# kjyv/FloBaRoID

Hardware: AMD Instinct MI355X
Metric: regressor samples/s (fused regressor->Gram pass) + TSQR TFLOP/s, WALK-MAN 31-DOF float-base (higher is better)
Workload: dtype f64

## Files before the change

flobaroid_amd/csrc/fbr_gram64.h:

```cpp
#pragma once
#define FBR_G64_SWZ(c) (2 * ((c) & 15))
#include <algorithm>
#include <type_traits>
#include <utility>

#include "fbr_kinid.h"

struct FbrGram64Tile {
    int col[FBR_TILE];
    std::vector<int> path;
    int friction = 0;
    int lo = 0, hi = 0;
};

struct FbrGram64 {
    int NT = 0;
    int NF = 0;
    int nlev = 0, fb = 0, flev = 0, ntr = 0, maxact = 0, npw = 0, wpb = 8;
    long blk_doubles = 0;
    std::vector<int> trow;
    std::vector<int> slab;
    int nstage = 0, base_stages = 0;
    std::vector<int> stage_lev;
    std::vector<int> lev_begin;
// ... 444 lines not shown
        for (int pq = 0; pq < pr.nparts; pq++)
            if (own[pq][l]) {
                pr.rel[((size_t)pq * hm.L + l) * FBR_G64_WORDS + 14 + p] = word(tr0, sl);
                pr.lcol[(size_t)pr.nparts * 10 * hm.L + ((size_t)pq * hm.L + l) * FBR_G64_FRIC + p] = c;
            }
    }
    pr.steps.clear();
    pr.nslots = 1;
    for (int pq = 0; pq < pr.nparts; pq++) {
        pr.step0[pq] = (int)(pr.steps.size() / FBR_KINID_STEP);
        pr.nsteps[pq] = progs[pq].nsteps;
        pr.nslots = std::max(pr.nslots, progs[pq].nslots);
        pr.steps.insert(pr.steps.end(), progs[pq].steps.begin(), progs[pq].steps.begin() + (size_t)progs[pq].nsteps * FBR_KINID_STEP);
    }
    return true;
}

static inline bool fbr_gram64_build_producer(const FbrHostModel &hm, const FbrGramProgram &, const FbrGram64 &g, FbrGram64Producer &pr)
{
    return fbr_gram64_build_producer(hm, g, pr);
}

#define FBR_G64_MAXK 2
FBR_HD int fbr_gram64_mom_count(int cols, int k) { return k * cols + k * (k + 1) / 2; }
FBR_HD void fbr_gram64_mom_target(int cols, int k, int idx, int *row, int *col)
{
    if (idx < k * cols) {
        *row = idx % cols;
        *col = cols + idx / cols;
        return;
    }
    int e = idx - k * cols, i = 0;
    while (e >= k - i) e -= k - i, i++;
    *row = cols + i;
    *col = cols + i + e;
}

#if defined(__HIPCC__) && defined(FBR_KERNELS_GRAM)
struct DevGram64 {
    int NT, nlev, maxact, npieces, nstage;
    long blk_doubles;
    const int *slab, *lev_begin, *pieces, *wmeta, *stage_lev;
    const int *runs;
};

template <int MAXD, bool HASW, int KR = 1>
__global__ __launch_bounds__(64 * FBR_KINWRITE_PARTS, MAXD <= 10 ? 2 : 1) void fbr_kinimg_kernel(DevModel m, DevKinId p, DevKinWrite wr, long S, long blk_doubles,
                                                                              const double *__restrict__ q, const double *__restrict__ dq,
                                                                              const double *__restrict__ ddq, const double *__restrict__ bv,
                                                                              const double *__restrict__ ba, const double *__restrict__ rpy,
                                                                              const double *__restrict__ rhs, const double *__restrict__ wts,
                                                                              double *__restrict__ scratch, double *__restrict__ mom,
                                                                              const double *__restrict__ sign)
{
    extern __shared__ __attribute__((aligned(16))) double smem[];
    const int lane = threadIdx.x & 63, part = __builtin_amdgcn_readfirstlane(threadIdx.x >> 6), nth = blockDim.x, tid = threadIdx.x;
    const int n = m.n, ldn = p.ldn, ldw = m.rows | 1, rows = m.rows;
    double *sq = smem, *sdq = sq + 64 * ldn, *sddq = sdq + 64 * ldn, *sw = sddq + 64 * ldn;
    double *st = sw + (HASW ? 64 * ldw : 0);
    double *scr = scratch + ((long)blockIdx.x * wr.nparts + part) * p.nslots * FBR_LINK_REC * 64 + lane;
    double *mo = mom ? mom + (long)blockIdx.x * (KR * wr.cols + KR * (KR + 1) / 2) * 64 : nullptr;
    const long Sg = wr.group_samples > 0 ? wr.group_samples : S, bpg = (Sg + 63) >> 6;
    const long nblk = (S / Sg) * bpg;
    const fbr_clong_ptr cdst = (fbr_clong_ptr)(unsigned long)wr.dst;
    const fbr_cint_ptr ccol = (fbr_cint_ptr)(unsigned long)(wr.lcol10 + (long)part * 10 * m.L);
    for (long blk = blockIdx.x; blk < nblk; blk += gridDim.x) {
        const long grp = blk / bpg, lb = blk - grp * bpg;
        const long base = grp * Sg + (lb << 6);
        const int valid = (int)min(64L, Sg - (lb << 6));
        __syncthreads();
        {
            const long off = base * n;
            const int cnt = valid * n;
            int sr = tid / n, dc = tid - sr * n;
            const int ds = nth / n, dd = nth - ds * n;
            for (int i = tid; i < cnt; i += nth) {
                const double a = q[off + i], b = dq[off + i], c = ddq[off + i];
                sq[sr * ldn + dc] = a;
                sdq[sr * ldn + dc] = b;
                sddq[sr * ldn + dc] = c;
                sr += ds;
                dc += dd;
                if (dc >= n) {
                    dc -= n;
                    sr++;
                }
            }
            if (HASW || wr.k) {
// ... 32 lines not shown
        };
        auto basest = [&](double *v6, double *a6, double *e3) {
            for (int i = 0; i < 6; i++) {
                v6[i] = bv[s * 6 + i];
                a6[i] = ba[s * 6 + i];
            }
            for (int i = 0; i < 3; i++) e3[i] = rpy[s * 3 + i];
        };
        auto save = [&](int b, int i, double v) { scr[(b * FBR_LINK_REC + i) * 64] = v; };
        auto load = [&](int b, int i) { return scr[(b * FBR_LINK_REC + i) * 64]; };
        auto consts = [&](int l, double *rR, double *rp, double *ax) {
            const fbr_cdouble_ptr cR = (fbr_cdouble_ptr)(unsigned long)m.restR, cp = (fbr_cdouble_ptr)(unsigned long)m.restp,
                                  ca = (fbr_cdouble_ptr)(unsigned long)m.axis;
            for (int i = 0; i < 9; i++) rR[i] = cR[9 * l + i];
            for (int i = 0; i < 3; i++) {
                rp[i] = cp[3 * l + i];
                ax[i] = ca[3 * l + i];
            }
        };
        const unsigned vlane = (unsigned)(((unsigned long)slot_off + (unsigned long)s31) << 3);
        auto link = [&](int l, int depth, const double *rec, const double (*Sst)[6], const int *lvd, double *F) {
            (void)F;
            if (wr.base_only) depth = 0;
            __builtin_amdgcn_s_waitcnt(0x0F70);
            long d10[10], dF[4];
#pragma unroll
            for (int pp = 0; pp < 10; pp++) d10[pp] = cdst[((long)part * m.L + l) * FBR_G64_WORDS + pp];
#pragma unroll
            for (int pp = 0; pp < 4; pp++) dF[pp] = cdst[((long)part * m.L + l) * FBR_G64_WORDS + 10 + pp];
            auto ft_of = [&](int ro, double *F) {
#pragma unroll
                for (int i = 0; i < 6; i++)
                    if (i < m.fb) F[i] = myt[ro + i];
#pragma unroll
                for (int j = 0; j < MAXD; j++)
                    if (j < depth) {
                        const double tj = myt[ro + m.fb + lvd[j]];
#pragma unroll
                        for (int i = 0; i < 6; i++) F[i] += Sst[j][i] * tj;
                    }
            };
            double Ft[6] = {0.0, 0.0, 0.0, 0.0, 0.0, 0.0};
            if constexpr (KR == 1) {
                if (wr.k) {
#pragma unroll
                    for (int i = 0; i < 6; i++)
                        if (i < m.fb) Ft[i] = myt[i];
#pragma unroll
                    for (int j = 0; j < MAXD; j++)
                        if (j < depth) {
                            const double tj = myt[m.fb + lvd[j]];
#pragma unroll
                            for (int i = 0; i < 6; i++) Ft[i] += Sst[j][i] * tj;
                        }
                }
            }
            auto ft_group = [&](int r, double *F) {
                int ro = r * 64 * ldw;
                asm volatile("" : "+v"(ro));
#pragma unroll
                for (int i = 0; i < 6; i++) F[i] = 0.0;
                ft_of(ro, F);
            };
            auto store = [&](long d0, int lv, double v) {
                if (d0 == 0) return;
                const unsigned vo = vlane ^ ((unsigned)(d0 & 0xff) << 3);
                __builtin_nontemporal_store(v, (fbr_gdouble_ptr)((fbr_gchar_ptr)(d0 & ~0xffL) + (long)lv * 8192 + vo));
            };
            auto full_group = [&](auto q0c, auto nqc) {
                constexpr int Q0 = decltype(q0c)::value, NQ = decltype(nqc)::value;
                double wA[NQ][6];
#pragma unroll
                for (int qq = 0; qq < NQ; qq++) fbr_unit_wrench(rec, Q0 + qq, wA[qq]);
#pragma unroll
                for (int i = 0; i < 6; i++)
                    if (i < m.fb) {
#pragma unroll
                        for (int qq = 0; qq < NQ; qq++) store(i < wr.flev ? dF[Q0 + qq] : d10[Q0 + qq], i, HASW ? wA[qq][i] * myw[i] : wA[qq][i]);
                    }
#pragma unroll
                for (int j = 0; j < MAXD; j++)
                    if (j < depth) {
                        double v[NQ];
#pragma unroll
                        for (int qq = 0; qq < NQ; qq++) v[qq] = fbr_dot6(Sst[j], wA[qq]);
                        const double wj = HASW ? myw[m.fb + lvd[j]] : 1.0;
#pragma unroll
                        for (int qq = 0; qq < NQ; qq++) store(d10[Q0 + qq], m.fb + j, HASW ? v[qq] * wj : v[qq]);
                    }
                if constexpr (KR == 1) {
                    if (wr.k) {
#pragma unroll
                        for (int qq = 0; qq < NQ; qq++)
                            if (d10[Q0 + qq]) unsafeAtomicAdd(mo + (long)ccol[10 * l + Q0 + qq] * 64 + lane, fbr_dot6(Ft, wA[qq]));
                    }
                } else {
#pragma unroll
                    for (int r = 0; r < KR; r++) {
                        double F[6];
                        ft_group(r, F);
#pragma unroll
                        for (int qq = 0; qq < NQ; qq++)
                            if (d10[Q0 + qq]) unsafeAtomicAdd(mo + ((long)r * wr.cols + ccol[10 * l + Q0 + qq]) * 64 + lane, fbr_dot6(F, wA[qq]));
                    }
                }
            };
            auto moment_group = [&](auto q0c, auto nqc) {
                constexpr int Q0 = decltype(q0c)::value, NQ = decltype(nqc)::value;
                double nB[NQ][3];
#pragma unroll
                for (int qq = 0; qq < NQ; qq++) fbr_unit_moment3(rec, 4 + Q0 + qq, nB[qq]);
#pragma unroll
                for (int i = 3; i < 6; i++)
                    if (i < m.fb) {
#pragma unroll
                        for (int qq = 0; qq < NQ; qq++) store(d10[4 + Q0 + qq], i, HASW ? nB[qq][i - 3] * myw[i] : nB[qq][i - 3]);
                    }
#pragma unroll
                for (int j = 0; j < MAXD; j++)
                    if (j < depth) {
                        double v[NQ];
#pragma unroll
                        for (int qq = 0; qq < NQ; qq++) v[qq] = Sst[j][3] * nB[qq][0] + Sst[j][4] * nB[qq][1] + Sst[j][5] * nB[qq][2];
                        const double wj = HASW ? myw[m.fb + lvd[j]] : 1.0;
#pragma unroll
                        for (int qq = 0; qq < NQ; qq++) store(d10[4 + Q0 + qq], m.fb + j, HASW ? v[qq] * wj : v[qq]);
                    }
                if constexpr (KR == 1) {
                    if (wr.k) {
#pragma unroll
                        for (int qq = 0; qq < NQ; qq++)
                            if (d10[4 + Q0 + qq])
                                unsafeAtomicAdd(mo + (long)ccol[10 * l + 4 + Q0 + qq] * 64 + lane, Ft[3] * nB[qq][0] + Ft[4] * nB[qq][1] + Ft[5] * nB[qq][2]);
                    }
                } else {
#pragma unroll
                    for (int r = 0; r < KR; r++) {
                        double F[6];
                        ft_group(r, F);
#pragma unroll
                        for (int qq = 0; qq < NQ; qq++)
                            if (d10[4 + Q0 + qq])
                                unsafeAtomicAdd(mo + ((long)r * wr.cols + ccol[10 * l + 4 + Q0 + qq]) * 64 + lane,
                                                F[3] * nB[qq][0] + F[4] * nB[qq][1] + F[5] * nB[qq][2]);
                    }
                }
            };
            using std::integral_constant;
            if constexpr (MAXD > 8 && MAXD <= 10) {
                full_group(integral_constant<int, 0>{}, integral_constant<int, 2>{});
                full_group(integral_constant<int, 2>{}, integral_constant<int, 2>{});
                moment_group(integral_constant<int, 0>{}, integral_constant<int, 3>{});
                moment_group(integral_constant<int, 3>{}, integral_constant<int, 3>{});
            } else {
                full_group(integral_constant<int, 0>{}, integral_constant<int, 4>{});
                moment_group(integral_constant<int, 0>{}, integral_constant<int, 6>{});
            }
            const int nfr = wr.cols > wr.ninert ? (wr.cols - wr.ninert) / n : 0;
            const int dj = nfr ? m.dof[l] : -1;
            if (dj >= 0 && depth > 0) {
                const fbr_cint_ptr cfr = (fbr_cint_ptr)(unsigned long)(wr.lcol10 + (long)wr.nparts * 10 * m.L + ((long)part * m.L + l) * FBR_G64_FRIC);
#pragma unroll
                for (int pf = 0; pf < FBR_G64_FRIC; pf++)
                    if (pf < nfr) {
                        const long dfw = cdst[((long)part * m.L + l) * FBR_G64_WORDS + 14 + pf];
                        if (dfw == 0) continue;
                        const int c = cfr[pf];
                        const double fv = fbr_friction_value(m.coldesc[c].z, mysdq[dj], sign ? sign[s * n + dj] : 0.0, m.stribeck);
                        store(dfw, m.fb + depth - 1, HASW ? fv * myw[m.fb + dj] : fv);
                        if constexpr (KR == 1) {
                            if (wr.k) unsafeAtomicAdd(mo + (long)c * 64 + lane, fv * myt[m.fb + dj]);
                        } else {
#pragma unroll
                            for (int r = 0; r < KR; r++) unsafeAtomicAdd(mo + ((long)r * wr.cols + c) * 64 + lane, fv * myt[r * 64 * ldw + m.fb + dj]);
                        }
                    }
            }
        };
        auto emit = [&](int, double) {};
        if (live) {
            fbr_kinid_lane<MAXD, false>(wr.part_nsteps[part], p.maxlvl, p.steps + wr.part_step0[part] * FBR_KINID_STEP, p.endflush, m.floating, m.g, m.fb,
                                        state, basest, save, load, link, emit, consts);
            if constexpr (KR == 1) {
                if (wr.k && part == wr.nparts - 1) {
                    double tt = 0.0;
                    for (int r = 0; r < rows; r++) {
                        const double wv = HASW ? myw[r] : 1.0, tv = rhs[s * rows + r] * wv;
                        tt += tv * tv;
                    }
                    unsafeAtomicAdd(mo + (long)wr.cols * 64 + lane, tt);
                }
            } else if (part == wr.nparts - 1) {
                double tt[KR * (KR + 1) / 2];
#pragma unroll
                for (int e = 0; e < KR * (KR + 1) / 2; e++) tt[e] = 0.0;
                for (int r = 0; r < rows; r++) {
                    const double wv = HASW ? myw[r] : 1.0;
                    double tv[KR];
#pragma unroll
                    for (int i = 0; i < KR; i++) tv[i] = rhs[(s * rows + r) * KR + i] * wv;
#pragma unroll
                    for (int i = 0, e = 0; i < KR; i++)
#pragma unroll
                        for (int j = i; j < KR; j++, e++) tt[e] += tv[i] * tv[j];
                }
#pragma unroll
                for (int e = 0; e < KR * (KR + 1) / 2; e++) unsafeAtomicAdd(mo + ((long)KR * wr.cols + e) * 64 + lane, tt[e]);
            }
        }
    }
}

__global__ __launch_bounds__(256) void fbr_gram64_tail_zero_kernel(double *__restrict__ img, long blk_doubles, long bpg, int ntr, int valid)
{
    double *blk = img + ((long)blockIdx.y * bpg + bpg - 1) * blk_doubles;
    const int per = 16 * (64 - valid);
    for (long e = (long)blockIdx.x * blockDim.x + threadIdx.x; e < (long)ntr * per; e += (long)gridDim.x * blockDim.x) {
        const int tr = (int)(e / per), r = (int)(e - (long)tr * per), c = r / (64 - valid), sl = valid + r % (64 - valid);
        blk[(long)tr * 1024 + (sl >> 5) * 512 + c * 32 + ((sl & 31) ^ FBR_G64_SWZ(c))] = 0.0;
    }
}

__global__ __launch_bounds__(256) void fbr_gram64_mom_reduce_kernel(int P, int k, int nwg, const double *__restrict__ mom, double *__restrict__ G)
{
    __shared__ double part[256];
    const int c = blockIdx.x, t = threadIdx.x, nm = fbr_gram64_mom_count(P, k);
    double s0 = 0.0, s1 = 0.0, s2 = 0.0, s3 = 0.0;
    int i = t;
    for (; i + 768 < nwg * 64; i += 1024) {
        s0 += mom[((long)(i >> 6) * nm + c) * 64 + (i & 63)];
        s1 += mom[((long)((i + 256) >> 6) * nm + c) * 64 + ((i + 256) & 63)];
        s2 += mom[((long)((i + 512) >> 6) * nm + c) * 64 + ((i + 512) & 63)];
        s3 += mom[((long)((i + 768) >> 6) * nm + c) * 64 + ((i + 768) & 63)];
    }
    for (; i < nwg * 64; i += 256) s0 += mom[((long)(i >> 6) * nm + c) * 64 + (i & 63)];
    part[t] = (s0 + s1) + (s2 + s3);
    __syncthreads();
    for (int o = 128; o > 0; o >>= 1) {
        if (t < o) part[t] += part[t + o];
        __syncthreads();
    }
    if (t) return;
    const int Pa = P + k;
    int row, col;
    fbr_gram64_mom_target(P, k, c, &row, &col);
    G[(long)row * Pa + col] += part[0];
    if (row != col) G[(long)col * Pa + row] += part[0];
}

template <int NPW, int WPB, bool RUNS = false>
__global__ __launch_bounds__(WPB * 64, (NPW <= 10) ? 4 : 2) void fbr_gram64_kernel(DevGram64 g, long nblk, const double *__restrict__ img,
                                                                                  double *__restrict__ partial, int carry)
{
    constexpr int MW = 3 * NPW;
    static_assert(MW <= 64, "a wave's slot table is fetched with one load");
    extern __shared__ __attribute__((aligned(16))) double smem[];
    const int bufd = g.maxact * 512;
    double *buf0 = smem, *buf1 = smem + bufd;
    int *slab = (int *)(smem + 2 * bufd);
    int *levb = slab + g.nlev * g.NT;
    int *pcs = levb + g.nlev + 1;
    int *wm = pcs + 2 * g.npieces;
    int *rn = wm + WPB * MW;
    static_assert(!RUNS || NPW > 10, "the 128-register shapes walk every slot");
    int *stl = rn + (RUNS ? WPB * g.nlev : 0);
    const int tid = threadIdx.x, lane = tid & 63;
    const int wave = __builtin_amdgcn_readfirstlane(tid >> 6);
    for (int i = tid; i < g.nlev * g.NT; i += WPB * 64) slab[i] = g.slab[i] * 512;
    for (int i = tid; i <= g.nlev; i += WPB * 64) levb[i] = g.lev_begin[i];
    for (int i = tid; i < 2 * g.npieces; i += WPB * 64) pcs[i] = g.pieces[i];
// ... 184 lines not shown
```

flobaroid_amd/csrc/fbr_gram_api.hip:

```cpp
#define FBR_KERNELS_GRAM
#include "fbr_internal.h"

static int get_deal(GramHolder *h, int wpg, GramHolder::Deal *out, bool base_only = false)
{
    const int key = wpg | (base_only ? 1 << 24 : 0);
    auto it = h->deals.find(key);
    if (it != h->deals.end()) {
        *out = it->second;
        return FBR_OK;
    }
    const std::vector<int> n = fbr_gram_deal(h->prog, wpg, base_only);
    std::vector<int2> tab;
    std::vector<int> begin(h->prog.T + 1, 0), given(h->prog.T, 0);
    for (int p = 0; p < h->prog.T; p++) begin[p + 1] = begin[p] + n[p];
    while ((int)tab.size() < begin[h->prog.T])
        for (int p = 0; p < h->prog.T; p++)
            if (given[p] < n[p]) tab.push_back(make_int2(p, given[p]++ | (n[p] << 16)));
    GramHolder::Deal d;
    int rc;
    if ((rc = upload(h->pool, tab, &d.tab))) return rc;
    if ((rc = upload(h->pool, begin, &d.begin))) return rc;
    h->deals[key] = d;
    *out = d;
    return FBR_OK;
// ... 242 lines not shown
    return finish_output(m, G, G_out, cnt, out_mem);
}
static size_t gram64_plds(const FbrHostModel &hm, int k, bool has_w)
{
    return ((size_t)3 * 64 * (std::max(hm.n, 1) | 1) + (size_t)((has_w ? 1 : 0) + k) * 64 * (hm.rows | 1)) * sizeof(double);
}

static int get_gram64(fbr_model *m, GramHolder *h)
{
    if (h->g64_state) return FBR_OK;
    h->g64_state = -1;
    const FbrHostModel &hm = m->hm;
    if (m->kinid.nsteps <= 0 || !fbr_gram64_build(hm, h->prog, h->g64, m->opt.gram_force_tiles != 0, m->opt.gram_lane_waves >= 16,
                                                         (int)m->opt.gram_lane_tiling))
        return FBR_OK;
    FbrGram64 &g = h->g64;
    if (fbr_gram64_lds_bytes(g) > FBR_G64_LDS_MAX) return FBR_OK;
    if (gram64_plds(hm, h->prog.k, true) > 160 * 1024) return FBR_OK;
    if (!fbr_gram64_build_producer(hm, g, h->g64p)) return FBR_OK;
    std::vector<int> wgbegin{0, 0};
    int rc;
    if ((rc = upload(h->pool, g.slab, &h->d64_slab)) || (rc = upload(h->pool, g.lev_begin, &h->d64_levb)) || (rc = upload(h->pool, g.pieces, &h->d64_pieces)) ||
        (rc = upload(h->pool, g.wmeta, &h->d64_wmeta)) || (rc = upload(h->pool, h->g64p.lcol, &h->d64_lcol)) ||
        (rc = upload(h->pool, h->g64p.steps, &h->d64_steps)) ||
        (rc = upload(h->pool, g.slot_tiles, &h->d64_slot_tiles)) || (rc = upload(h->pool, g.tilecol, &h->d64_tilecol)) ||
        (rc = upload(h->pool, g.stage_lev, &h->d64_stagelev)) || (!g.runs.empty() && (rc = upload(h->pool, g.runs, &h->d64_runs))))
        return rc;
    h->g64_state = 1;
    return FBR_OK;
}

static int gram64_serves(fbr_model *m, GramHolder *h, int k, bool *serves)
{
    *serves = false;
    if (!m->opt.gram_lane || k > FBR_G64_MAXK || (k > 0 && !h->moments)) return FBR_OK;
    if (int rc = get_gram64(m, h)) return rc;
    *serves = h->g64_state == 1;
    return FBR_OK;
}

static long gram64_chunk_blocks(const FbrGram64 &g) { return std::max<long>(1, (long)((size_t)3 * 1024 * 1024 * 1024 / ((size_t)g.blk_doubles * 8))); }

static int gram64_wg_table(GramHolder *h, int wgs, const int **out)
{
    auto it = h->d64_wb.find(wgs);
    if (it == h->d64_wb.end()) {
// ... 47 lines not shown
    dg.maxact = g.maxact;
    dg.npieces = (int)g.pieces.size() / 2;
    dg.blk_doubles = g.blk_doubles;
    dg.slab = h->d64_slab;
    dg.lev_begin = h->d64_levb;
    dg.pieces = h->d64_pieces;
    dg.wmeta = h->d64_wmeta;
    dg.nstage = base_only ? g.base_stages : g.nstage;
    dg.stage_lev = h->d64_stagelev;
    dg.runs = g.runs.empty() ? nullptr : h->d64_runs;
    L->gk = g.wpb == 16 ? fbr_gram64_kernel<10, 16>
            : g.npw == 10   ? fbr_gram64_kernel<10, 8>
            : g.runs.empty() ? fbr_gram64_kernel<FBR_ONE_SEGW * FBR_ONE_NSEG, 8> : fbr_gram64_kernel<FBR_ONE_SEGW * FBR_ONE_NSEG, 8, true>;
    L->glds = fbr_gram64_lds_bytes(g);
    L->vnpw = g.npw * (g.wpb / 8);
    HIPCHK(hipFuncSetAttribute((const void *)L->gk, hipFuncAttributeMaxDynamicSharedMemorySize, (int)L->glds));
    return FBR_OK;
}

static DevKinWrite gram64_kinwrite(const fbr_model *m, const GramHolder *h, int b, int k, bool has_w, bool base_only, long group_samples)
{
    DevKinWrite kw{};
    kw.lcol10 = h->d64_lcol;
    kw.dst = (const long *)h->dst64[b].p;
    kw.ninert = m->hm.ninert;
    kw.cols = m->hm.cols;
    kw.k = k;
    kw.has_w = has_w ? 1 : 0;
    kw.flev = h->g64.flev;
    kw.base_only = base_only ? 1 : 0;
    kw.group_samples = group_samples;
    kw.nparts = h->g64p.nparts;
    for (int pq = 0; pq < FBR_KINWRITE_PARTS; pq++) {
        kw.part_nsteps[pq] = h->g64p.nsteps[pq];
        kw.part_step0[pq] = h->g64p.step0[pq];
    }
    return kw;
}

static int gram64_produce(fbr_model *m, GramHolder *h, const Gram64Launch &L, const DevKinWrite &kw, int pblocks, size_t plds, long cs,
                          const DevStates &d, long so, const double *rhs, int k, const double *w, double *mom)
{
    const FbrHostModel &hm = m->hm;
    return kinimg_by_depth(m, [&](auto D) -> int {
        const auto kernel = k == 2 ? (kw.has_w ? fbr_kinimg_kernel<D, true, 2> : fbr_kinimg_kernel<D, false, 2>)
                                   : (kw.has_w ? fbr_kinimg_kernel<D, true> : fbr_kinimg_kernel<D, false>);
// ... 65 lines not shown

static int gram64_pass(fbr_model *m, GramHolder *h, const DevStates &d, const double *drhs, const double *dw, int k, double *G, bool base_only,
                       bool h2d_chunked)
{
    const FbrHostModel &hm = m->hm;
    const FbrGram64 &g = h->g64;
    const long S = d.S;
    int rc;
    const long nblocks = (S + 63) / 64;
    long chb = gram64_chunk_blocks(g);
    if (h2d_chunked) chb = std::min<long>(chb, 7L * m->num_cus);
    if (m->opt.chunk_samples >= 1) chb = std::min(gram64_chunk_blocks(g), std::max<long>(1, ((long)m->opt.chunk_samples + 63) / 64));
    chb = std::min(nblocks, chb);
    if (chb < nblocks && chb > m->num_cus) chb = chb / m->num_cus * m->num_cus;
    long chs = chb * 64;
    if (m->opt.chunk_samples >= 1) chs = std::min(chs, (long)m->opt.chunk_samples);
    if ((rc = gram64_ensure_images(m, h, chb))) return rc;
    Gram64Launch L;
    if ((rc = gram64_setup(m, h, base_only, &L))) return rc;
    const size_t plds = gram64_plds(hm, k, dw != nullptr);
    const int pblocks = (int)std::min<long>(chb, (long)L.pgrid_max);
    const int gwgs = (int)std::min<long>(chb, (long)m->num_cus);
    if (k) {
        if ((rc = h->mom64.ensure((size_t)L.pgrid_max * fbr_gram64_mom_count(hm.cols, k) * 64 * sizeof(double)))) return rc;
        HIPCHK(hipMemsetAsync(h->mom64.p, 0, (size_t)pblocks * fbr_gram64_mom_count(hm.cols, k) * 64 * sizeof(double), m->stream));
    }
    if ((rc = m->partial.ensure((size_t)m->num_cus * g.wpb * g.npw * 256 * sizeof(double)))) return rc;
    int launches = 0, first_wgs = 0;
    if (h2d_chunked) {
        if ((rc = ensure_stage_buffers(m, d, k, dw, chs, 2)) || (rc = ensure_copy_stream(m))) return rc;
        HIPCHK(hipEventRecord(m->ev_fork, m->stream));
    }
    struct Staged {
        DevStates dc;
        long o;
        const double *rhs, *w;
    };
    auto stage = [&](long c, Staged &out) -> int {
        const long s0 = c * chs, cs = std::min(chs, S - s0);
        const int b = (int)(c & 1);
        out = {d, s0, drhs, dw};
        if (!h2d_chunked) return FBR_OK;
        HIPCHK(hipStreamWaitEvent(m->copy, m->ev_pack_rec[b] ? m->ev_pack[b] : m->ev_fork, 0));
        ProfScope ps(m, FBR_PROF_H2D, m->copy);
        if (int r3 = stage_chunk(m, d, drhs, k, dw, s0, cs, b, m->copy, &out.dc, &out.rhs, &out.w)) return r3;
        out.o = 0;
        HIPCHK(hipEventRecord(m->ev_h2d[b], m->copy));
        return FBR_OK;
    };
    Staged cur, nxt;
    if (S > 0 && (rc = stage(0, nxt))) return rc;
    for (long s0 = 0; s0 < S; s0 += chs, launches++) {
        const long cs = std::min(chs, S - s0), nb = (cs + 63) / 64;
        const int b = launches & 1;
        cur = nxt;
        if (s0 + chs < S && (rc = stage(launches + 1, nxt))) return rc;
        if (h2d_chunked) HIPCHK(hipStreamWaitEvent(m->stream, m->ev_h2d[b], 0));
        if (cs & 63)
            HIPCHK(hipMemsetAsync(h->img64[b].as<double>() + (nb - 1) * g.blk_doubles, 0, (size_t)g.blk_doubles * sizeof(double), m->stream));
        {
            ProfScope ps(m, FBR_PROF_PACK);
            if ((rc = gram64_produce(m, h, L, gram64_kinwrite(m, h, b, k, dw != nullptr, base_only, 0), pblocks, plds, cs, cur.dc, cur.o, cur.rhs, k,
                                     cur.w, k ? h->mom64.as<double>() : nullptr)))
                return rc;
            if (h2d_chunked) {
                HIPCHK(hipEventRecord(m->ev_pack[b], m->stream));
                m->ev_pack_rec[b] = true;
            }
        }
        const int wgs = (int)std::min<long>(nb, (long)gwgs);
        if (launches == 0) first_wgs = wgs;
        if (wgs > first_wgs) {
            set_err("internal: Gram launch wider than the first one of the call");
            return FBR_E_INVALID;
        }
        {
            ProfScope ps(m, FBR_PROF_GRAM);
            hipLaunchKernelGGL(L.gk, dim3(first_wgs), dim3(g.wpb * 64), L.glds, m->stream, L.dg, nb, h->img64[b].as<double>(), m->partial.as<double>(),
                               launches > 0 ? 1 : 0);
            HIPCHK(hipGetLastError());
        }
    }
    if (launches > 0) {
        ProfScope ps(m, FBR_PROF_REDUCE);
        const int *wgb = nullptr;
        if ((rc = gram64_wg_table(h, first_wgs, &wgb)) || (rc = gram64_reduce(m, h, L, first_wgs, wgb, 1, G))) return rc;
        if (k) {
            hipLaunchKernelGGL(fbr_gram64_mom_reduce_kernel, dim3(fbr_gram64_mom_count(hm.cols, k)), dim3(256), 0, m->stream, hm.cols, k, pblocks,
                               h->mom64.as<double>(), G);
            HIPCHK(hipGetLastError());
        }
    }
    return FBR_OK;
}

static int gram64_grouped_pass(fbr_model *m, GramHolder *h, const DevStates &d, const double *dw, double *G, int ngroups)
{
    const FbrHostModel &hm = m->hm;
    const FbrGram64 &g = h->g64;
    const long S = d.S, Sg = S / ngroups, bpg = (Sg + 63) / 64;
    const int Pa = hm.cols;
    int rc;
    const int gpc = (int)std::min<long>(std::min(ngroups, 32768), std::max<long>(1, gram64_chunk_blocks(g) / bpg));
    if ((rc = gram64_ensure_images(m, h, (long)gpc * bpg))) return rc;
    const int wpg = (int)std::max<long>(1, std::min<long>(bpg, (long)m->num_cus / std::min(gpc, ngroups)));
    Gram64Launch L;
    if ((rc = gram64_setup(m, h, false, &L))) return rc;
    const size_t plds = gram64_plds(hm, 0, dw != nullptr);
    if ((rc = m->partial.ensure((size_t)gpc * wpg * g.wpb * g.npw * 256 * sizeof(double)))) return rc;
    const int *wgb = nullptr;
    if ((rc = gram64_wg_table(h, wpg, &wgb))) return rc;
    for (int g0 = 0, launches = 0; g0 < ngroups; g0 += gpc, launches++) {
        const int ng = std::min(gpc, ngroups - g0), b = launches & 1;
        const long s0 = (long)g0 * Sg, cs = (long)ng * Sg, nb = (long)ng * bpg;
        if (Sg & 63) {
            hipLaunchKernelGGL(fbr_gram64_tail_zero_kernel, dim3(16, ng), dim3(256), 0, m->stream, h->img64[b].as<double>(), g.blk_doubles, bpg, g.ntr, (int)(Sg & 63));
            HIPCHK(hipGetLastError());
        }
        {
            ProfScope ps(m, FBR_PROF_PACK);
            if ((rc = gram64_produce(m, h, L, gram64_kinwrite(m, h, b, 0, dw != nullptr, false, Sg), (int)std::min<long>(nb, (long)L.pgrid_max), plds, cs,
                                     d, s0, nullptr, 0, dw, nullptr)))
                return rc;
        }
        {
            ProfScope ps(m, FBR_PROF_GRAM);
            hipLaunchKernelGGL(L.gk, dim3(wpg, ng), dim3(g.wpb * 64), L.glds, m->stream, L.dg, bpg, h->img64[b].as<double>(), m->partial.as<double>(), 0);
            HIPCHK(hipGetLastError());
        }
        {
            ProfScope ps(m, FBR_PROF_REDUCE);
            if ((rc = gram64_reduce(m, h, L, wpg, wgb, ng, G + (size_t)g0 * Pa * Pa))) return rc;
        }
    }
    return FBR_OK;
}

static int print_gram_timing(fbr_model *m, int T, const unsigned long long *dbg, int NW)
{
    std::vector<unsigned long long> hb((size_t)NW * FBR_WPB * 8);
    HIPCHK(hipMemcpyAsync(hb.data(), dbg, hb.size() * sizeof(unsigned long long), hipMemcpyDeviceToHost, m->stream));
    HIPCHK(hipStreamSynchronize(m->stream));
    static const char *names[3] = {"wait_dma+barrier", "dma_issue", "mfma"};
    std::vector<double> sum((size_t)T * 3, 0.0), ns(T, 0.0), nw(T, 0.0), wv((size_t)T * FBR_WPB, 0.0);
    for (size_t e = 0; e + 8 <= hb.size(); e += 8) {
        const int part = (int)hb[e + 6];
// ... 375 lines not shown
```

flobaroid_amd/csrc/fbr_internal.h:

```cpp
#pragma once
#include <hip/hip_runtime.h>
#include <unistd.h>

#include <algorithm>
#include <cstdint>
#include <cstdio>
#include <cstdlib>
#include <cstring>
#include <map>
#include <memory>
#include <numeric>
#include <string>
#include <vector>

#include "../../include/fbr.h"
#include "fbr_options.h"
#include "fbr_kernels.h"
#include "fbr_kinid.h"
#include "fbr_capsule.h"
#include "fbr_capsule_grad.h"
#include "fbr_gram64.h"
#include "fbr_tsqr_work.h"
#include "fbr_weights.h"

// ... 61 lines not shown
    DevBuf &b = pool.back();
    size_t n = std::max<size_t>(v.size(), 1) * sizeof(T);
    int rc = b.ensure(n);
    if (rc) return rc;
    if (!v.empty()) HIPCHK(hipMemcpy(b.p, v.data(), v.size() * sizeof(T), hipMemcpyHostToDevice));
    *out = (const T *)b.p;
    return FBR_OK;
}

struct GramHolder {
    FbrGramProgram prog;
    DevGram dev;
    std::vector<DevBuf> pool;
    DevBuf pimg[2];
    bool moments = false;
    DevBuf mom[2];
    bool mom_clean[2] = {false, false};
    const int *itemcol = nullptr;
    size_t lds_bytes = 0;
    size_t pack_lds_bytes = 0;
    int g64_state = 0;
    FbrGram64 g64;
    FbrGram64Producer g64p;
    const int *d64_slab = nullptr, *d64_levb = nullptr, *d64_pieces = nullptr, *d64_wmeta = nullptr, *d64_lcol = nullptr,
              *d64_steps = nullptr, *d64_slot_tiles = nullptr, *d64_tilecol = nullptr, *d64_stagelev = nullptr,
              *d64_runs = nullptr;
    DevBuf img64[2], dst64[2], mom64, scr64;
    long img64_blocks = 0;
    std::map<int, const int *> d64_wb;
    struct Deal { const int2 *tab; const int *begin; };
    std::map<int, Deal> deals;
};

struct fbr_model {
    FbrOptions opt;
    FbrHostModel hm;
    DevModel dm;
    int device = 0;
    pid_t pid = 0;
    int num_cus = 256;
    hipStream_t own_stream = nullptr, stream = nullptr;
    hipStream_t side = nullptr;
    hipStream_t copy = nullptr;
    hipEvent_t ev_pack[2] = {nullptr, nullptr}, ev_gram[2] = {nullptr, nullptr}, ev_fork = nullptr, ev_h2d[2] = {nullptr, nullptr};
    hipEvent_t ev_done[2] = {nullptr, nullptr};
    int64_t next_ticket = 0;
    int64_t waited_ticket = -1;
// ... 170 lines not shown
```

flobaroid_amd/csrc/fbr_kinid.h:

```cpp
#pragma once
#include <type_traits>
#include <vector>

#include "fbr_math.h"
#include "fbr_program.h"

#define FBR_KINID_STEP 8
#define FBR_KINID_MAXD 24

#define FBR_KINWRITE_PARTS 4

template <int D, int... Ds, class F> inline auto fbr_by_depth(int maxlvl, F &&f)
{
    if constexpr (sizeof...(Ds) > 0)
        if (maxlvl > D) return fbr_by_depth<Ds...>(maxlvl, f);
    return f(std::integral_constant<int, D>());
}

#if defined(__HIPCC__)
typedef const __attribute__((address_space(4))) long *fbr_clong_ptr;
typedef const __attribute__((address_space(4))) int *fbr_cint_ptr;
typedef const __attribute__((address_space(4))) double *fbr_cdouble_ptr;
#endif

// ... 189 lines not shown
    int nsteps, maxlvl, nslots, ldn;
    const int *steps, *endflush;
};
struct DevKinExt {
    long T, tiles, nblk;
    double *val;
    long *idx;
};
FBR_HD double fbr_ext_value(int k, double v)
{
    if (k == 2) return fabs(v);
    if (k == 3) return v != v ? 0.0 : fmin(fabs(v), 1.7976931348623157e308);
    return v;
}
FBR_HD bool fbr_ext_take(int k, double a, double b)
{
    if (b != b) return false;
    return a != a || (k == 0 ? a < b : a > b);
}
typedef __attribute__((address_space(1))) char *fbr_gchar_ptr;
typedef __attribute__((address_space(1))) double *fbr_gdouble_ptr;
struct DevKinWrite {
    const int *lcol10, *colrec;
    const long *dst;
    int ninert, cols, k, has_w;
    int flev;
    int base_only;
    long group_samples;
    int nparts, part_nsteps[FBR_KINWRITE_PARTS], part_step0[FBR_KINWRITE_PARTS];
};
#endif

#if defined(__HIPCC__) && defined(FBR_KERNELS_CORE)

template <int MAXD, bool EXT = false>
__global__ __launch_bounds__(64) void fbr_kinid_kernel(DevModel m, DevKinId p, long S, const double *__restrict__ q, const double *__restrict__ dq,
                                                       const double *__restrict__ ddq, const double *__restrict__ bv,
                                                       const double *__restrict__ ba, const double *__restrict__ rpy,
                                                       const double *__restrict__ sign, const double *__restrict__ vel_sign,
                                                       const double *__restrict__ x, int mode, double *__restrict__ tau, double *__restrict__ scratch, int flink, double fpx,
                                                       double fpy, double fpz, DevKinExt ex)
{
    extern __shared__ __attribute__((aligned(16))) double smem[];
    const int lane = threadIdx.x, n = m.n, ldn = p.ldn;
    double *sq = smem, *sdq = sq + 64 * ldn, *sddq = sdq + 64 * ldn;
    double *scr = scratch + (long)blockIdx.x * p.nslots * FBR_LINK_REC * 64 + lane;
// ... 385 lines not shown
```

Before: 86.48 million.

## Reduce moment accumulators across lanes before atomics instead of per-lane slots

Moment (regressor-times-rhs) contributions used to be atomically added into a per-lane slot for every column, so the buffer was 64x larger and needed a wide reduction. Now each wavefront sums its lanes with permlane swaps and DPP shuffles, each lane is assigned one target column from a precomputed lane-column table, and a single atomic per lane is issued. The moment buffer, its memset, and the reduce kernel shrink to match. Tail-zero launches also move after the producer. In exchange, extra cross-lane shuffles run on every link even when a column is absent, and the lane mapping adds complexity and correctness risk.

```diff
diff --git a/flobaroid_amd/csrc/fbr_gram64.h b/flobaroid_amd/csrc/fbr_gram64.h
--- a/flobaroid_amd/csrc/fbr_gram64.h
+++ b/flobaroid_amd/csrc/fbr_gram64.h
@@ -490,6 +490,7 @@
 }
 
 #define FBR_G64_MAXK 2
+#include "fbr_mom_lanes.h"
 FBR_HD int fbr_gram64_mom_count(int cols, int k) { return k * cols + k * (k + 1) / 2; }
 FBR_HD void fbr_gram64_mom_target(int cols, int k, int idx, int *row, int *col)
 {
@@ -504,7 +505,64 @@
     *col = cols + i + e;
 }
 
+#define FBR_G64_LANECOL_RHS 24
+static inline std::vector<int> fbr_gram64_lane_columns(const FbrGram64Producer &pr, int L)
+{
+    std::vector<int> t((size_t)pr.nparts * L * 64, -1);
+    for (int pq = 0; pq < pr.nparts; pq++)
+        for (int l = 0; l < L; l++)
+            for (int r = 0; r < FBR_G64_MAXK; r++) {
+                int *row = &t[((size_t)pq * L + l) * 64];
+                for (int p = 0; p < 10; p++) {
+                    const int c = pr.lcol[((size_t)pq * L + l) * 10 + p];
+                    if (c >= 0) row[fbr_gram64_mom_lane(p, r)] = c | r << FBR_G64_LANECOL_RHS;
+                }
+                for (int pf = 0; pf < FBR_G64_FRIC; pf++) {
+                    const int c = pr.lcol[(size_t)pr.nparts * 10 * L + ((size_t)pq * L + l) * FBR_G64_FRIC + pf];
+                    if (c >= 0) row[fbr_gram64_mom_fric_lane(pf, r)] = c | r << FBR_G64_LANECOL_RHS;
+                }
+            }
+    return t;
+}
+
 #if defined(__HIPCC__) && defined(FBR_KERNELS_GRAM)
+struct FbrMomLanesDev {
+    int lane;
+    template <int CTRL>
+    static __device__ __forceinline__ double dpp(double v)
+    {
+        const long b = __builtin_bit_cast(long, v);
+        const int lo = __builtin_amdgcn_update_dpp(0, (int)b, CTRL, 0xf, 0xf, true), hi = __builtin_amdgcn_update_dpp(0, (int)(b >> 32), CTRL, 0xf, 0xf, true);
+        return __builtin_bit_cast(double, ((long)(unsigned)hi << 32) | (long)(unsigned)lo);
+    }
+    static __device__ __forceinline__ void put(double &a, double &b, unsigned l0, unsigned l1, unsigned h0, unsigned h1)
+    {
+        a = __builtin_bit_cast(double, ((long)h0 << 32) | (long)l0);
+        b = __builtin_bit_cast(double, ((long)h1 << 32) | (long)l1);
+    }
+    __device__ __forceinline__ void swap32(double &a, double &b) const
+    {
+        const long x = __builtin_bit_cast(long, a), y = __builtin_bit_cast(long, b);
+        const auto l = __builtin_amdgcn_permlane32_swap((unsigned)x, (unsigned)y, false, false);
+        const auto h = __builtin_amdgcn_permlane32_swap((unsigned)(x >> 32), (unsigned)(y >> 32), false, false);
+        put(a, b, l[0], l[1], h[0], h[1]);
+    }
+    __device__ __forceinline__ void swap16(double &a, double &b) const
+    {
+        const long x = __builtin_bit_cast(long, a), y = __builtin_bit_cast(long, b);
+        const auto l = __builtin_amdgcn_permlane16_swap((unsigned)x, (unsigned)y, false, false);
+        const auto h = __builtin_amdgcn_permlane16_swap((unsigned)(x >> 32), (unsigned)(y >> 32), false, false);
+        put(a, b, l[0], l[1], h[0], h[1]);
+    }
+    __device__ __forceinline__ double get8(double a) const { return dpp<0x128>(a); }
+    __device__ __forceinline__ double get7(double a) const { return dpp<0x141>(a); }
+    __device__ __forceinline__ double get2(double a) const { return dpp<0x4E>(a); }
+    __device__ __forceinline__ double get1(double a) const { return dpp<0xB1>(a); }
+    __device__ __forceinline__ double live0(bool live, double a) const { return live ? a : 0.0; }
+    __device__ __forceinline__ double bit8(double a, double b) const { return (lane & 8) ? b : a; }
+    __device__ __forceinline__ double zero() const { return 0.0; }
+};
+
 struct DevGram64 {
     int NT, nlev, maxact, npieces, nstage;
     long blk_doubles;
@@ -527,11 +585,13 @@
     double *sq = smem, *sdq = sq + 64 * ldn, *sddq = sdq + 64 * ldn, *sw = sddq + 64 * ldn;
     double *st = sw + (HASW ? 64 * ldw : 0);
     double *scr = scratch + ((long)blockIdx.x * wr.nparts + part) * p.nslots * FBR_LINK_REC * 64 + lane;
-    double *mo = mom ? mom + (long)blockIdx.x * (KR * wr.cols + KR * (KR + 1) / 2) * 64 : nullptr;
+    double *mo = mom ? mom + (long)blockIdx.x * (KR * wr.cols + KR * (KR + 1) / 2) : nullptr;
+    const bool domom = KR > 1 || wr.k != 0;
+    const FbrMomLanesDev mx{lane};
     const long Sg = wr.group_samples > 0 ? wr.group_samples : S, bpg = (Sg + 63) >> 6;
     const long nblk = (S / Sg) * bpg;
     const fbr_clong_ptr cdst = (fbr_clong_ptr)(unsigned long)wr.dst;
-    const fbr_cint_ptr ccol = (fbr_cint_ptr)(unsigned long)(wr.lcol10 + (long)part * 10 * m.L);
+    const __attribute__((address_space(1))) int *glcol = (const __attribute__((address_space(1))) int *)(unsigned long)wr.lanecol + (long)part * m.L * 64 + lane;
     for (long blk = blockIdx.x; blk < nblk; blk += gridDim.x) {
         const long grp = blk / bpg, lb = blk - grp * bpg;
         const long base = grp * Sg + (lb << 6);
@@ -610,7 +670,18 @@
         auto link = [&](int l, int depth, const double *rec, const double (*Sst)[6], const int *lvd, double *F) {
             (void)F;
             if (wr.base_only) depth = 0;
+            int mycol = -1;
+            if (domom) mycol = glcol[l * 64];
             __builtin_amdgcn_s_waitcnt(0x0F70);
+            double macc = 0.0;
+            auto mom_sum = [&](auto g0c, auto ngc, auto p0c, auto nqc, const double *v, int r) {
+                constexpr int G0 = decltype(g0c)::value, NG = decltype(ngc)::value, P0 = decltype(p0c)::value, NQ = decltype(nqc)::value;
+                double u[NG];
+#pragma unroll
+                for (int i = 0; i < NG; i++) u[i] = (G0 + i >= P0 && G0 + i < P0 + NQ) ? v[G0 + i - P0] : 0.0;
+                const double sum = fbr_mom_lanes_sum<NG>(u, live, mx);
+                if (G0 == 0 ? (lane & 15) == 6 * r : (lane & 7) == 1 + 6 * r) macc += sum;
+            };
             long d10[10], dF[4];
 #pragma unroll
             for (int pp = 0; pp < 10; pp++) d10[pp] = cdst[((long)part * m.L + l) * FBR_G64_WORDS + pp];
@@ -650,6 +721,7 @@
                 for (int i = 0; i < 6; i++) F[i] = 0.0;
                 ft_of(ro, F);
             };
+            using std::integral_constant;
             auto store = [&](long d0, int lv, double v) {
                 if (d0 == 0) return;
                 const unsigned vo = vlane ^ ((unsigned)(d0 & 0xff) << 3);
@@ -676,20 +748,23 @@
 #pragma unroll
                         for (int qq = 0; qq < NQ; qq++) store(d10[Q0 + qq], m.fb + j, HASW ? v[qq] * wj : v[qq]);
                     }
+                long any = 0;
+#pragma unroll
+                for (int qq = 0; qq < NQ; qq++) any |= d10[Q0 + qq];
+                if (!domom || any == 0) return;
+                double v[NQ];
                 if constexpr (KR == 1) {
-                    if (wr.k) {
-#pragma unroll
-                        for (int qq = 0; qq < NQ; qq++)
-                            if (d10[Q0 + qq]) unsafeAtomicAdd(mo + (long)ccol[10 * l + Q0 + qq] * 64 + lane, fbr_dot6(Ft, wA[qq]));
-                    }
+#pragma unroll
+                    for (int qq = 0; qq < NQ; qq++) v[qq] = fbr_dot6(Ft, wA[qq]);
+                    mom_sum(integral_constant<int, 0>{}, integral_constant<int, 4>{}, q0c, nqc, v, 0);
                 } else {
 #pragma unroll
                     for (int r = 0; r < KR; r++) {
                         double F[6];
                         ft_group(r, F);
 #pragma unroll
-                        for (int qq = 0; qq < NQ; qq++)
-                            if (d10[Q0 + qq]) unsafeAtomicAdd(mo + ((long)r * wr.cols + ccol[10 * l + Q0 + qq]) * 64 + lane, fbr_dot6(F, wA[qq]));
+                        for (int qq = 0; qq < NQ; qq++) v[qq] = fbr_dot6(F, wA[qq]);
+                        mom_sum(integral_constant<int, 0>{}, integral_constant<int, 4>{}, q0c, nqc, v, r);
                     }
                 }
             };
@@ -714,27 +789,26 @@
 #pragma unroll
                         for (int qq = 0; qq < NQ; qq++) store(d10[4 + Q0 + qq], m.fb + j, HASW ? v[qq] * wj : v[qq]);
                     }
+                long any = 0;
+#pragma unroll
+                for (int qq = 0; qq < NQ; qq++) any |= d10[4 + Q0 + qq];
+                if (!domom || any == 0) return;
+                double v[NQ];
                 if constexpr (KR == 1) {
-                    if (wr.k) {
-#pragma unroll
-                        for (int qq = 0; qq < NQ; qq++)
-                            if (d10[4 + Q0 + qq])
-                                unsafeAtomicAdd(mo + (long)ccol[10 * l + 4 + Q0 + qq] * 64 + lane, Ft[3] * nB[qq][0] + Ft[4] * nB[qq][1] + Ft[5] * nB[qq][2]);
-                    }
+#pragma unroll
+                    for (int qq = 0; qq < NQ; qq++) v[qq] = Ft[3] * nB[qq][0] + Ft[4] * nB[qq][1] + Ft[5] * nB[qq][2];
+                    mom_sum(integral_constant<int, 4>{}, integral_constant<int, 6>{}, integral_constant<int, 4 + Q0>{}, nqc, v, 0);
                 } else {
 #pragma unroll
                     for (int r = 0; r < KR; r++) {
                         double F[6];
                         ft_group(r, F);
 #pragma unroll
-                        for (int qq = 0; qq < NQ; qq++)
-                            if (d10[4 + Q0 + qq])
-                                unsafeAtomicAdd(mo + ((long)r * wr.cols + ccol[10 * l + 4 + Q0 + qq]) * 64 + lane,
-                                                F[3] * nB[qq][0] + F[4] * nB[qq][1] + F[5] * nB[qq][2]);
+                        for (int qq = 0; qq < NQ; qq++) v[qq] = F[3] * nB[qq][0] + F[4] * nB[qq][1] + F[5] * nB[qq][2];
+                        mom_sum(integral_constant<int, 4>{}, integral_constant<int, 6>{}, integral_constant<int, 4 + Q0>{}, nqc, v, r);
                     }
                 }
             };
-            using std::integral_constant;
             if constexpr (MAXD > 8 && MAXD <= 10) {
                 full_group(integral_constant<int, 0>{}, integral_constant<int, 2>{});
                 full_group(integral_constant<int, 2>{}, integral_constant<int, 2>{});
@@ -756,17 +830,19 @@
                         const int c = cfr[pf];
                         const double fv = fbr_friction_value(m.coldesc[c].z, mysdq[dj], sign ? sign[s * n + dj] : 0.0, m.stribeck);
                         store(dfw, m.fb + depth - 1, HASW ? fv * myw[m.fb + dj] : fv);
-                        if constexpr (KR == 1) {
-                            if (wr.k) unsafeAtomicAdd(mo + (long)c * 64 + lane, fv * myt[m.fb + dj]);
-                        } else {
-#pragma unroll
-                            for (int r = 0; r < KR; r++) unsafeAtomicAdd(mo + ((long)r * wr.cols + c) * 64 + lane, fv * myt[r * 64 * ldw + m.fb + dj]);
+                        if (!domom) continue;
+#pragma unroll
+                        for (int r = 0; r < KR; r++) {
+                            const double v = fv * myt[r * 64 * ldw + m.fb + dj], sum = fbr_mom_lanes_sum<1>(&v, live, mx);
+                            if (lane == fbr_gram64_mom_fric_lane(pf, r)) macc = sum;
                         }
                     }
             }
+            if (domom && mycol >= 0 && (KR > 1 || mycol < (1 << FBR_G64_LANECOL_RHS)))
+                unsafeAtomicAdd(mo + (mycol >> FBR_G64_LANECOL_RHS) * wr.cols + (mycol & ((1 << FBR_G64_LANECOL_RHS) - 1)), macc);
         };
         auto emit = [&](int, double) {};
-        if (live) {
+        {
             fbr_kinid_lane<MAXD, false>(wr.part_nsteps[part], p.maxlvl, p.steps + wr.part_step0[part] * FBR_KINID_STEP, p.endflush, m.floating, m.g, m.fb,
                                         state, basest, save, load, link, emit, consts);
             if constexpr (KR == 1) {
@@ -776,7 +852,8 @@
                         const double wv = HASW ? myw[r] : 1.0, tv = rhs[s * rows + r] * wv;
                         tt += tv * tv;
                     }
-                    unsafeAtomicAdd(mo + (long)wr.cols * 64 + lane, tt);
+                    const double sum = fbr_mom_lanes_sum<1>(&tt, live, mx);
+                    if (lane == 0) unsafeAtomicAdd(mo + wr.cols, sum);
                 }
             } else if (part == wr.nparts - 1) {
                 double tt[KR * (KR + 1) / 2];
@@ -792,8 +869,13 @@
 #pragma unroll
                         for (int j = i; j < KR; j++, e++) tt[e] += tv[i] * tv[j];
                 }
-#pragma unroll
-                for (int e = 0; e < KR * (KR + 1) / 2; e++) unsafeAtomicAdd(mo + ((long)KR * wr.cols + e) * 64 + lane, tt[e]);
+                double mine = 0.0;
+#pragma unroll
+                for (int e = 0; e < KR * (KR + 1) / 2; e++) {
+                    const double sum = fbr_mom_lanes_sum<1>(&tt[e], live, mx);
+                    if (lane == e) mine = sum;
+                }
+                if (lane < KR * (KR + 1) / 2) unsafeAtomicAdd(mo + (long)KR * wr.cols + lane, mine);
             }
         }
     }
@@ -811,29 +893,31 @@
 
 __global__ __launch_bounds__(256) void fbr_gram64_mom_reduce_kernel(int P, int k, int nwg, const double *__restrict__ mom, double *__restrict__ G)
 {
-    __shared__ double part[256];
-    const int c = blockIdx.x, t = threadIdx.x, nm = fbr_gram64_mom_count(P, k);
+    __shared__ double part[4][64];
+    const int w = threadIdx.x >> 6, t = threadIdx.x & 63, nm = fbr_gram64_mom_count(P, k), c = blockIdx.x * 4 + w;
     double s0 = 0.0, s1 = 0.0, s2 = 0.0, s3 = 0.0;
-    int i = t;
-    for (; i + 768 < nwg * 64; i += 1024) {
-        s0 += mom[((long)(i >> 6) * nm + c) * 64 + (i & 63)];
-        s1 += mom[((long)((i + 256) >> 6) * nm + c) * 64 + ((i + 256) & 63)];
-        s2 += mom[((long)((i + 512) >> 6) * nm + c) * 64 + ((i + 512) & 63)];
-        s3 += mom[((long)((i + 768) >> 6) * nm + c) * 64 + ((i + 768) & 63)];
-    }
-    for (; i < nwg * 64; i += 256) s0 += mom[((long)(i >> 6) * nm + c) * 64 + (i & 63)];
-    part[t] = (s0 + s1) + (s2 + s3);
+    if (c < nm) {
+        int i = t;
+        for (; i + 192 < nwg; i += 256) {
+            s0 += mom[(long)i * nm + c];
+            s1 += mom[(long)(i + 64) * nm + c];
+            s2 += mom[(long)(i + 128) * nm + c];
+            s3 += mom[(long)(i + 192) * nm + c];
+        }
+        for (; i < nwg; i += 64) s0 += mom[(long)i * nm + c];
+    }
+    part[w][t] = (s0 + s1) + (s2 + s3);
     __syncthreads();
-    for (int o = 128; o > 0; o >>= 1) {
-        if (t < o) part[t] += part[t + o];
+    for (int o = 32; o > 0; o >>= 1) {
+        if (t < o) part[w][t] += part[w][t + o];
         __syncthreads();
     }
-    if (t) return;
+    if (t || c >= nm) return;
     const int Pa = P + k;
     int row, col;
     fbr_gram64_mom_target(P, k, c, &row, &col);
-    G[(long)row * Pa + col] += part[0];
-    if (row != col) G[(long)col * Pa + row] += part[0];
+    G[(long)row * Pa + col] += part[w][0];
+    if (row != col) G[(long)col * Pa + row] += part[w][0];
 }
 
 template <int NPW, int WPB, bool RUNS = false>
diff --git a/flobaroid_amd/csrc/fbr_gram_api.hip b/flobaroid_amd/csrc/fbr_gram_api.hip
--- a/flobaroid_amd/csrc/fbr_gram_api.hip
+++ b/flobaroid_amd/csrc/fbr_gram_api.hip
@@ -288,6 +288,7 @@
     int rc;
     if ((rc = upload(h->pool, g.slab, &h->d64_slab)) || (rc = upload(h->pool, g.lev_begin, &h->d64_levb)) || (rc = upload(h->pool, g.pieces, &h->d64_pieces)) ||
         (rc = upload(h->pool, g.wmeta, &h->d64_wmeta)) || (rc = upload(h->pool, h->g64p.lcol, &h->d64_lcol)) ||
+        (rc = upload(h->pool, fbr_gram64_lane_columns(h->g64p, hm.L), &h->d64_lanecol)) ||
         (rc = upload(h->pool, h->g64p.steps, &h->d64_steps)) ||
         (rc = upload(h->pool, g.slot_tiles, &h->d64_slot_tiles)) || (rc = upload(h->pool, g.tilecol, &h->d64_tilecol)) ||
         (rc = upload(h->pool, g.stage_lev, &h->d64_stagelev)) || (!g.runs.empty() && (rc = upload(h->pool, g.runs, &h->d64_runs))))
@@ -381,6 +382,7 @@
 {
     DevKinWrite kw{};
     kw.lcol10 = h->d64_lcol;
+    kw.lanecol = h->d64_lanecol;
     kw.dst = (const long *)h->dst64[b].p;
     kw.ninert = m->hm.ninert;
     kw.cols = m->hm.cols;
@@ -492,8 +494,8 @@
     const int pblocks = (int)std::min<long>(chb, (long)L.pgrid_max);
     const int gwgs = (int)std::min<long>(chb, (long)m->num_cus);
     if (k) {
-        if ((rc = h->mom64.ensure((size_t)L.pgrid_max * fbr_gram64_mom_count(hm.cols, k) * 64 * sizeof(double)))) return rc;
-        HIPCHK(hipMemsetAsync(h->mom64.p, 0, (size_t)pblocks * fbr_gram64_mom_count(hm.cols, k) * 64 * sizeof(double), m->stream));
+        if ((rc = h->mom64.ensure((size_t)L.pgrid_max * fbr_gram64_mom_count(hm.cols, k) * sizeof(double)))) return rc;
+        HIPCHK(hipMemsetAsync(h->mom64.p, 0, (size_t)pblocks * fbr_gram64_mom_count(hm.cols, k) * sizeof(double), m->stream));
     }
     if ((rc = m->partial.ensure((size_t)m->num_cus * g.wpb * g.npw * 256 * sizeof(double)))) return rc;
     int launches = 0, first_wgs = 0;
@@ -526,13 +528,15 @@
         cur = nxt;
         if (s0 + chs < S && (rc = stage(launches + 1, nxt))) return rc;
         if (h2d_chunked) HIPCHK(hipStreamWaitEvent(m->stream, m->ev_h2d[b], 0));
-        if (cs & 63)
-            HIPCHK(hipMemsetAsync(h->img64[b].as<double>() + (nb - 1) * g.blk_doubles, 0, (size_t)g.blk_doubles * sizeof(double), m->stream));
         {
             ProfScope ps(m, FBR_PROF_PACK);
             if ((rc = gram64_produce(m, h, L, gram64_kinwrite(m, h, b, k, dw != nullptr, base_only, 0), pblocks, plds, cs, cur.dc, cur.o, cur.rhs, k,
                                      cur.w, k ? h->mom64.as<double>() : nullptr)))
                 return rc;
+            if (cs & 63) {
+                hipLaunchKernelGGL(fbr_gram64_tail_zero_kernel, dim3(16, 1), dim3(256), 0, m->stream, h->img64[b].as<double>(), g.blk_doubles, nb, g.ntr, (int)(cs & 63));
+                HIPCHK(hipGetLastError());
+            }
             if (h2d_chunked) {
                 HIPCHK(hipEventRecord(m->ev_pack[b], m->stream));
                 m->ev_pack_rec[b] = true;
@@ -556,7 +560,7 @@
         const int *wgb = nullptr;
         if ((rc = gram64_wg_table(h, first_wgs, &wgb)) || (rc = gram64_reduce(m, h, L, first_wgs, wgb, 1, G))) return rc;
         if (k) {
-            hipLaunchKernelGGL(fbr_gram64_mom_reduce_kernel, dim3(fbr_gram64_mom_count(hm.cols, k)), dim3(256), 0, m->stream, hm.cols, k, pblocks,
+            hipLaunchKernelGGL(fbr_gram64_mom_reduce_kernel, dim3((fbr_gram64_mom_count(hm.cols, k) + 3) / 4), dim3(256), 0, m->stream, hm.cols, k, pblocks,
                                h->mom64.as<double>(), G);
             HIPCHK(hipGetLastError());
         }
@@ -583,15 +587,15 @@
     for (int g0 = 0, launches = 0; g0 < ngroups; g0 += gpc, launches++) {
         const int ng = std::min(gpc, ngroups - g0), b = launches & 1;
         const long s0 = (long)g0 * Sg, cs = (long)ng * Sg, nb = (long)ng * bpg;
-        if (Sg & 63) {
-            hipLaunchKernelGGL(fbr_gram64_tail_zero_kernel, dim3(16, ng), dim3(256), 0, m->stream, h->img64[b].as<double>(), g.blk_doubles, bpg, g.ntr, (int)(Sg & 63));
-            HIPCHK(hipGetLastError());
-        }
         {
             ProfScope ps(m, FBR_PROF_PACK);
             if ((rc = gram64_produce(m, h, L, gram64_kinwrite(m, h, b, 0, dw != nullptr, false, Sg), (int)std::min<long>(nb, (long)L.pgrid_max), plds, cs,
                                      d, s0, nullptr, 0, dw, nullptr)))
                 return rc;
+            if (Sg & 63) {
+                hipLaunchKernelGGL(fbr_gram64_tail_zero_kernel, dim3(16, ng), dim3(256), 0, m->stream, h->img64[b].as<double>(), g.blk_doubles, bpg, g.ntr, (int)(Sg & 63));
+                HIPCHK(hipGetLastError());
+            }
         }
         {
             ProfScope ps(m, FBR_PROF_GRAM);
diff --git a/flobaroid_amd/csrc/fbr_internal.h b/flobaroid_amd/csrc/fbr_internal.h
--- a/flobaroid_amd/csrc/fbr_internal.h
+++ b/flobaroid_amd/csrc/fbr_internal.h
@@ -107,7 +107,7 @@
     int g64_state = 0;
     FbrGram64 g64;
     FbrGram64Producer g64p;
-    const int *d64_slab = nullptr, *d64_levb = nullptr, *d64_pieces = nullptr, *d64_wmeta = nullptr, *d64_lcol = nullptr,
+    const int *d64_slab = nullptr, *d64_levb = nullptr, *d64_pieces = nullptr, *d64_wmeta = nullptr, *d64_lcol = nullptr, *d64_lanecol = nullptr,
               *d64_steps = nullptr, *d64_slot_tiles = nullptr, *d64_tilecol = nullptr, *d64_stagelev = nullptr,
               *d64_runs = nullptr;
     DevBuf img64[2], dst64[2], mom64, scr64;
diff --git a/flobaroid_amd/csrc/fbr_kinid.h b/flobaroid_amd/csrc/fbr_kinid.h
--- a/flobaroid_amd/csrc/fbr_kinid.h
+++ b/flobaroid_amd/csrc/fbr_kinid.h
@@ -235,6 +235,7 @@
 typedef __attribute__((address_space(1))) double *fbr_gdouble_ptr;
 struct DevKinWrite {
     const int *lcol10, *colrec;
+    const int *lanecol = nullptr;
     const long *dst;
     int ninert, cols, k, has_w;
     int flev;
diff --git a/flobaroid_amd/csrc/fbr_mom_lanes.h b/flobaroid_amd/csrc/fbr_mom_lanes.h
--- /dev/null
+++ b/flobaroid_amd/csrc/fbr_mom_lanes.h
@@ -0,0 +1,59 @@
+#pragma once
+#include "fbr_math.h"
+
+FBR_HD int fbr_mom_lanes_class(int nq, int lane)
+{
+    const int h32 = (nq + 1) / 2, h16 = (h32 + 1) / 2;
+    const int i8 = h16 > 1 ? (lane >> 3) & 1 : 0;
+    const int i16 = h32 > 1 ? i8 + h16 * ((lane >> 4) & 1) : 0;
+    if (i16 >= h32) return -1;
+    const int c = nq > 1 ? i16 + h32 * ((lane >> 5) & 1) : 0;
+    return c < nq ? c : -1;
+}
+
+FBR_HD int fbr_gram64_mom_lane(int pidx, int r = 0)
+{
+    if (pidx < 4) return 16 * pidx + 6 * r;
+    const int q = pidx - 4;
+    return 32 * (q / 3) + 8 * (q % 3) + 1 + 6 * r;
+}
+FBR_HD int fbr_gram64_mom_fric_lane(int pf, int r = 0) { return 2 + pf + 8 * r; }
+
+template <int NQ, class T, class L, class X>
+FBR_HD T fbr_mom_lanes_sum(const T *v, const L &live, X &x)
+{
+    static_assert(NQ >= 1 && NQ <= 8, "two split exchanges and bit 8 tell at most eight columns apart");
+    constexpr int H32 = (NQ + 1) / 2, H16 = (H32 + 1) / 2;
+    T a[H32], b[H16];
+#if defined(__HIPCC__)
+#pragma unroll
+#endif
+    for (int i = 0; i < H32; i++) {
+        a[i] = x.live0(live, v[i]);
+        T up = i + H32 < NQ ? x.live0(live, v[i + H32]) : (NQ == 1 ? a[i] : x.zero());
+        x.swap32(a[i], up);
+        a[i] = a[i] + up;
+    }
+#if defined(__HIPCC__)
+#pragma unroll
+#endif
+    for (int i = 0; i < H16; i++) {
+        b[i] = a[i];
+        T up = i + H16 < H32 ? a[i + H16] : (H32 == 1 ? a[i] : x.zero());
+        x.swap16(b[i], up);
+        b[i] = b[i] + up;
+    }
+#if defined(__HIPCC__)
+#pragma unroll
+#endif
+    for (int i = 0; i < H16; i++) {
+        b[i] = b[i] + x.get8(b[i]);
+        b[i] = b[i] + x.get7(b[i]);
+        b[i] = b[i] + x.get2(b[i]);
+        b[i] = b[i] + x.get1(b[i]);
+    }
+    if constexpr (H16 > 1)
+        return x.bit8(b[0], b[1]);
+    else
+        return b[0];
+}
```

Result: faster. 88.73 million, median of 6 (+2.6%).
